# ndefilippis/SWRaytracing

Measured on AMD Instinct MI355X. Metric: packet-steps/sec @ 512² field, 1e6 packets; 1/2/4/8-GPU scaling, higher is better.
Workload: dtype f64

## Files before the change

### swraytracing_amd/csrc/swrt_host_packets.hpp

```cpp
#pragma once
#include <algorithm>
#include <vector>

#include "swrt_ctx.hpp"
#include "swrt_host_fields.hpp"
#include "swrt_bin.hpp"
#include "swrt_kernels.hpp"
#include "swrt_tile.hpp"
#include "swrt_share.hpp"
#include "swrt_xka.hpp"
#include "swrt_spectral.hpp"

namespace {

bool use_tile_kernel(const swrt_ctx* c) {
  if (c->rebin_every <= 0) return false;
  if (c->kernel == 2) return true;
  return c->kernel == 0 && c->slot[0].nx >= 2 * kTile;
}

bool tile_binned(const swrt_ctx* c) { return use_tile_kernel(c) && c->bin.tiled_for(tiles_per_side(c->slot[0].nx)); }

struct IvLaunch {
  int nint;
  FieldView views[kMaxIntervals + 1];
  double dts[kMaxIntervals];
  bool div_free;
};

template <typename F, typename... Args>
void launch_k(swrt_ctx* c, F kernel, dim3 grid, dim3 block, Args... args) {
  hipEvent_t stop = c->kev1 ? c->kev1 : (slot_events(c) ? c->use_ev.get() : nullptr);
  hipExtLaunchKernelGGL(kernel, grid, block, 0, c->stream, c->kev0, stop, 0, args...);
  c->tail_ev = stop;
}

constexpr int64_t kMultiStreamFrom = 65536;

int hz_tile_launch(swrt_ctx* c, const TileArgs& t, const TileShare* parts, int nparts, bool zero_counts,
                   bool fork = true) {
  HazardChecker h = c->hz;
  if (zero_counts) {
    const uint64_t tm = h.op(0);
    if (!h.access(0, tm, t.next_counts, kHzWrite, HzRegion::all(), "the next-binning counts' memset"))
      return fail(c, SWRT_ERR_STATE, h.err);
  }
  if (nparts > 1 && fork) {
    h.record(c->fork_ev.get(), 0);
    for (int i = 1; i < nparts; ++i) h.wait(i, c->fork_ev.get());
  }
  const StepArgs& a = t.s;
  for (int p = 0; p < nparts; ++p) {
    const uint64_t tp = h.op(p);
    const HzRegion r = HzRegion::of_share(h.epoch, parts[p]);
    const char* what = t.src ? "a part of the sort launch after a re-binning" : "a part launch";
    const HzRegion rin = t.src ? HzRegion::all() : r;
    bool ok = h.access(p, tp, a.x, kHzRead, rin, what) && h.access(p, tp, a.k, kHzRead, rin, what) &&
              h.access(p, tp, a.perm, kHzRead, rin, what) && h.access(p, tp, t.src, kHzRead, r, what) &&
              h.access(p, tp, t.starts, kHzRead, HzRegion::all(), what) &&
              h.access(p, tp, t.order, kHzRead, HzRegion::all(), what) &&
              h.access(p, tp, t.x_out, kHzWrite, r, what) && h.access(p, tp, t.k_out, kHzWrite, r, what) &&
              h.access(p, tp, t.perm_out, kHzWrite, r, what) &&
              h.access(p, tp, t.next_keys, kHzWrite, r, what) &&
              h.access(p, tp, t.next_counts, kHzAtomic, HzRegion::all(), what) &&
              h.access(p, tp, a.hist_x, kHzWrite, r, what) && h.access(p, tp, a.hist_k, kHzWrite, r, what);
    if (!ok) return fail(c, SWRT_ERR_STATE, h.err);
  }
  c->hz = std::move(h);
  return SWRT_OK;
}

int launch_tiles(swrt_ctx* c, void (*kernel)(TileArgs), int nt, TileArgs t, bool zero_counts) {
  const int ntiles = t.ntx * t.ntx;
  const int S = c->n >= kMultiStreamFrom ? c->packet_streams : 1;
  const bool skew = c->dbg.share_skew && t.next_keys != nullptr;
  if (skew && !c->hz.on) return fail(c, SWRT_ERR_STATE, "the skewed share runs only under the hazard checker");
  const bool multi = S == 2 && c->stream == c->stream0.get() && c->sx[0].get() != nullptr &&
                     (skew ? ntiles % 8 == 0 && ntiles / 8 >= 3 : ntiles % 16 == 0);
  if (!multi) {
    t.sh = TileShare{ntiles, -1, 1, kShareEven};
    HIPCHK_RC(join_b(c));
    if (c->hz.on) HIPCHK_RC(hz_tile_launch(c, t, &t.sh, 1, zero_counts));
    if (zero_counts) HIPCHK(c, hipMemsetAsync(t.next_counts, 0, sizeof(int) * ntiles, c->stream));
    launch_k(c, kernel, dim3((unsigned)share_grid(t.sh)), dim3(nt), t);
    c->s0_dirty = true;
    return SWRT_OK;
  }
  const TileShare sh[2] = {TileShare{ntiles, 0, 2, skew ? kShareSkew : kShareEven},
                           TileShare{ntiles, 1, 2, skew ? kShareSkew : kShareEven}};
  const bool fork = c->s0_dirty || zero_counts || skew;
  if (c->hz.on) HIPCHK_RC(hz_tile_launch(c, t, sh, 2, zero_counts, fork));
  if (zero_counts) HIPCHK(c, hipMemsetAsync(t.next_counts, 0, sizeof(int) * ntiles, c->stream));
  if (fork) {
    HIPCHK(c, hipEventRecord(c->fork_ev.get(), c->stream));
    HIPCHK(c, hipStreamWaitEvent(c->sx[0].get(), c->fork_ev.get(), 0));
  }
  c->s0_dirty = false;
  t.sh = sh[0];
  hipExtLaunchKernelGGL(kernel, dim3((unsigned)share_grid(sh[0])), dim3(nt), 0, c->stream, c->kev0, nullptr, 0, t);
  if (c->dbg.spin_us > 0)
    hipLaunchKernelGGL(debug_spin_kernel, dim3(1), dim3(64), 0, c->sx[0].get(), (c->dbg.spin_us + 3) / 4);
  t.sh = sh[1];
  hipExtLaunchKernelGGL(kernel, dim3((unsigned)share_grid(sh[1])), dim3(nt), 0, c->sx[0].get(), nullptr, c->kev1, 0, t);
  c->b_pending = 1;
  c->tail_ev = nullptr;
  return SWRT_OK;
}

bool sparse_tiles(const swrt_ctx* c, int64_t ntiles) {
  if (c->sparse_mode == 1) return false;
  if (c->sparse_mode == 2) return true;
  return c->n < (int64_t)kSparseBelow * ntiles;
}

int tile_threads(const swrt_ctx* c, bool v5_two, int64_t ntiles) {
  return v5_two && sparse_tiles(c, ntiles) ? kSparseThreads : kTileThreads;
}

bool two_v5(const swrt_ctx* c, int nslots, int sa) {
  bool v5 = nslots >= 2;
  for (int i = 0; i < nslots && v5; ++i) v5 = c->slot[sa + i].div_free;
  return v5;
}

int tile_cells(const swrt_ctx* c, int64_t nx) {
  if (use_tile_kernel(c)) return kTile;
  if (c->tile > 0) return (int)std::min<int64_t>(c->tile, nx);
  int t = 8;
  while ((nx + t - 1) / t > 64) t *= 2;
  return t;
}

using LeapKernel = void (*)(StepArgs);
LeapKernel leap_kernel(int nslots) { return nslots == 2 ? leapfrog_kernel<true> : leapfrog_kernel<false>; }

int rebin(swrt_ctx* c, bool indirect, int tile = 0, int lanes = kTileThreads) {
  if (int rc = join_b(c)) return rc;
  c->s0_dirty = true;
  const Slot& s = c->slot[0];
  const FieldView v = view_of(s);
  BinGeom g;
  g.dx = v.dx; g.px = v.px; g.py = v.py; g.inv_px = v.inv_px; g.inv_py = v.inv_py; g.inv_dx = v.inv_dx;
  g.nx = v.nx;
  g.tile = tile > 0 ? tile : tile_cells(c, s.nx);
  g.ntx = (int)((s.nx + g.tile - 1) / g.tile);
  const int nbins = g.ntx * g.ntx;
  if (nbins > kMaxBins) return fail(c, SWRT_ERR_ARG, "too many spatial bins (raise tile size)");
  const int64_t n = c->n;
  const unsigned grid = nblocks(n, 256 * kBinPerThread);
  const bool keys_valid = c->bin.keys_valid_for(nbins, v.nx, v.dx);
  const PacketSet &in = c->pk.cur, &out = c->pk.out;
  if (c->hz.on) {
    HazardChecker& h = c->hz;
    const uint64_t t = h.op(0);
    const char* what = "a re-binning";
    const bool ok =
        hz_whole(h, t, kHzRead, what, {in.x.get(), in.k.get(), in.perm.get()}) &&
        hz_whole(h, t, keys_valid ? kHzRead : kHzWrite, what, {c->keys.get()}) &&
        hz_whole(h, t, kHzWrite, what, {c->bins.counts(), c->bins.cursor(), c->bins.starts(), c->bins.tile_order()}) &&
        (indirect ? hz_whole(h, t, kHzWrite, what, {c->src_idx.get()})
                  : hz_whole(h, t, kHzWrite, what, {out.x.get(), out.k.get(), out.perm.get()}));
    if (!ok) return fail(c, SWRT_ERR_STATE, h.err);
    ++h.epoch;
  }
  if (!keys_valid) {
    if (c->bin.needs_count_memset(nbins))
      HIPCHK(c, hipMemsetAsync(c->bins.counts(), 0, sizeof(int) * nbins, c->stream));
    hipLaunchKernelGGL(bin_count_kernel, dim3(grid), dim3(256), sizeof(int) * nbins, c->stream, g, in.x.get(), n,
                       nbins, c->keys.get(), c->bins.counts());
    HIPCHK(c, hipGetLastError());
  }
  if (c->dbg.corrupt_count != 0) {
    hipLaunchKernelGGL(debug_corrupt_count_kernel, dim3(1), dim3(64), 0, c->stream, c->bins.counts(), nbins / 2,
                       c->dbg.corrupt_count);
    c->dbg.corrupt_count = 0;
  }
  hipLaunchKernelGGL(bin_scan_kernel, dim3(1), dim3(1024), 0, c->stream, c->bins.counts(), nbins, c->bins.cursor(),
                     c->bins.starts(), n, c->dev_err.dev(), c->bins.tile_order(), lanes);
  HIPCHK(c, hipGetLastError());
  hipLaunchKernelGGL(indirect ? bin_scatter_kernel<true> : bin_scatter_kernel<false>, dim3(grid), dim3(256),
                     2 * sizeof(int) * nbins, c->stream, in.x.get(), in.k.get(), in.perm.get(), c->keys.get(), n, nbins,
                     c->bins.cursor(), out.x.get(), out.k.get(), out.perm.get(), indirect ? c->src_idx.get() : nullptr);
  HIPCHK(c, hipGetLastError());
  if (!indirect) c->pk.flip();
  c->bin.rebinned(nbins, g.tile, lanes, indirect);
  return SWRT_OK;
}

struct TileKernel { void (*fn)(TileArgs); int threads; };
TileKernel tile_kernel_of(bool two, bool v5, bool fma, bool sparse) {
  constexpr int T = kTile, M = kMargin, NT = kTileThreads, ST = kSparseThreads, PF = kSparsePrefetch;
  constexpr int MW = kSparseMinWaves;
  if (two && v5 && sparse)
    return {fma ? tile_leapfrog_kernel<true, T, M, ST, true, true, PF, MW>
                : tile_leapfrog_kernel<true, T, M, ST, true, false, PF, MW>, ST};
  if (two && v5) return {fma ? tile_leapfrog_kernel<true, T, M, NT, true, true> : tile_leapfrog_kernel<true, T, M, NT, true>, NT};
  if (two) return {tile_leapfrog_kernel<true, T, M, NT>, NT};
  if (v5) return {fma ? tile_leapfrog_kernel<false, T, M, NT, true, true> : tile_leapfrog_kernel<false, T, M, NT, true>, NT};
  return {tile_leapfrog_kernel<false, T, M, NT>, NT};
}

int tile_launch(swrt_ctx* c, const StepArgs& a, bool count_next, const IvLaunch* iv = nullptr) {
  TileArgs t;
  t.s = a;
  t.ivmode = iv != nullptr;
  t.nint = iv ? iv->nint : 1;
  if (iv) {
    for (int i = 0; i <= iv->nint; ++i) t.ivn[i] = iv->views[i].nodes;
    for (int i = 0; i < iv->nint; ++i) t.ivdt[i] = iv->dts[i];
  }
  t.x_out = c->pk.out.x.get();
  t.k_out = c->pk.out.k.get();
  t.perm_out = c->pk.out.perm.get();
  t.starts = c->bins.starts();
  t.order = c->bins.tile_order();
  if (c->bin.tile() != kTile) return fail(c, SWRT_ERR_STATE, "the binning is not the LDS-tiled kernel's");
  t.ntx = tiles_per_side(a.f0.nx);
  const int ntiles = t.ntx * t.ntx;
  t.next_keys = nullptr;
  t.next_counts = nullptr;
  t.sort_cells = c->bin.cells_sorted() ? 0 : 1;
  t.src = nullptr;
  t.sort_lead = c->sort_lead ? 0.5 * a.dt * (double)std::max<int64_t>(1, c->rebin_every) : 0.0;
  if (c->bin.src_pending()) {
    t.src = c->src_idx.get();
    t.sort_cells = 1;
  }
  bool zero = false;
  if (count_next && ntiles == c->bin.nbins()) {
    zero = !c->bin.counts_zero();
    t.next_keys = c->keys.get();
    t.next_counts = c->bins.counts();
  }
  const bool two = a.nslots == 2;
  const bool v5 = two ? (iv ? iv->div_free : two_v5(c, 2, 0)) : c->slot[0].div_free;
  const TileKernel tk = tile_kernel_of(two, v5, c->gather_mode == 1,
                                       two && v5 && tile_threads(c, true, ntiles) == kSparseThreads);
  HIPCHK_RC(launch_tiles(c, tk.fn, tk.threads, t, zero));
  HIPCHK(c, hipGetLastError());
  c->bin.tile_launched(t.next_keys != nullptr, a.f0.nx, a.f0.dx);
  if (t.src != nullptr && c->b_pending && !c->dbg.legacy_park) {
    c->pk.park_cur();
  } else {
    c->pk.flip();
  }
  return SWRT_OK;
}

int leap_launch(swrt_ctx* c, const StepArgs& a, unsigned grid) {
  HIPCHK_RC(join_b(c));
  c->s0_dirty = true;
  if (c->hz.on) {
    HazardChecker& h = c->hz;
    const uint64_t t = h.op(0);
    const char* what = "the per-packet leapfrog launch";
    if (!(hz_whole(h, t, kHzWrite, what, {a.x, a.k}) && hz_whole(h, t, kHzRead, what, {a.perm}) &&
          hz_whole(h, t, kHzWrite, what, {a.hist_x, a.hist_k})))
      return fail(c, SWRT_ERR_STATE, h.err);
  }
  c->bin.per_packet_launched();
  if (c->kev1) {
    launch_k(c, leap_kernel(a.nslots), dim3(grid), dim3(256), a);
  } else {
    hipLaunchKernelGGL(leap_kernel(a.nslots), dim3(grid), dim3(256), 0, c->stream, a);
    c->tail_ev = nullptr;
  }
  HIPCHK(c, hipGetLastError());
  return SWRT_OK;
}

int timed_launch(swrt_ctx* c, const StepArgs& a, unsigned grid, bool count_next, const IvLaunch* iv = nullptr) {
  const bool timed = c->timing_every > 0 && (c->launch_count++ % c->timing_every) == 0;
  const auto launch = [&] { return use_tile_kernel(c) ? tile_launch(c, a, count_next, iv) : leap_launch(c, a, grid); };
  if (!timed) return launch();
  if (c->timing.used + 2 > kMaxEvents) {
    if (int rc = sync_sx(c)) return rc;
    HIPCHK(c, hipStreamSynchronize(c->stream));
    for (size_t i = 0; i + 1 < c->timing.used; i += 2) {
      float ms = 0.f;
      HIPCHK(c, hipEventElapsedTime(&ms, c->timing.ev[i].get(), c->timing.ev[i + 1].get()));
      c->timing.folded_ms += ms;
      c->timing.folded_n += 1;
    }
    c->timing.used = 0;
  }
  if (c->timing.used + 2 > c->timing.ev.size()) {
    for (int e = 0; e < 64; ++e) {
      Event ev;
      HIPCHK(c, ev.create(hipEventDefault));
      c->timing.ev.push_back(std::move(ev));
    }
  }
  c->kev0 = c->timing.ev[c->timing.used].get();
  c->kev1 = c->timing.ev[c->timing.used + 1].get();
  c->timing.used += 2;
  const int rc = launch();
  c->kev0 = c->kev1 = nullptr;
  return rc;
}

int leap_rebin_if_due(swrt_ctx* c, int nslots, int sa) {
  if (c->rebin_every <= 0) return SWRT_OK;
  const bool tiled = use_tile_kernel(c);
  const int64_t ntx = tiles_per_side(c->slot[sa].nx), ntiles = tiled ? ntx * ntx : 0;
  const int lanes = tiled ? tile_threads(c, two_v5(c, nslots, sa), ntiles) : kTileThreads;
  if (c->bin.due(c->rebin_every) || (tiled && (c->bin.tile() != kTile || c->bin.lanes() != lanes)))
    return rebin(c, tiled, tiled ? kTile : 0, lanes);
  return SWRT_OK;
}

StepArgs step_args(swrt_ctx* c, const FieldView& f0, const FieldView& f1, int nslots, double dt, double f, double gH,
                   double alpha0, double dalpha, double bump, int64_t save_every) {
  StepArgs a;
  a.f0 = f0;
  a.f1 = f1;
  a.nslots = nslots;
  a.n = c->n;
  a.dt = dt;
  a.half = dt / 2;
  a.f2 = f * f;
  a.fastdisp = dispersion_fast(a.f2);
  a.gH = gH;
  a.alpha0 = alpha0;
  a.dalpha = dalpha;
  a.bump = bump;
  a.save_every = save_every > 0 ? save_every : 1;
  a.hist_x = save_every > 0 ? c->hist.a.get() : nullptr;
  a.hist_k = save_every > 0 ? c->hist.b.get() : nullptr;
  a.frame0 = c->hist.ext.frames();
  return a;
}

int advance_launch(swrt_ctx* c, StepArgs& a, int64_t s0, int64_t nsteps, int64_t steps, const IvLaunch* iv = nullptr) {
  a.x = c->pk.cur.x.get();
  a.k = c->pk.cur.k.get();
  a.perm = c->pk.cur.perm.get();
  a.s0 = s0;
  a.nsteps = (int)nsteps;
  const bool count_next = c->rebin_every > 0 && steps >= c->bin.steps_left(c->rebin_every);
  slot_writes_wait(c);
  HIPCHK_RC(timed_launch(c, a, nblocks(c->n, 256), count_next, iv));
  c->bin.stepped(steps);
  return SWRT_OK;
}

int run_advance(swrt_ctx* c, double dt, int64_t nsteps, double f, double gH, int nslots,
                double alpha0, double dalpha, double bump, int64_t save_every, int sa = 0) {
  const FieldView f0 = view_of(c->slot[sa]);
  StepArgs a = step_args(c, f0, nslots == 2 ? view_of(c->slot[sa + 1]) : f0, nslots, dt, f, gH, alpha0, dalpha, bump,
                         save_every);
  int64_t s0 = 0;
  while (s0 < nsteps) {
    int64_t chunk = std::min<int64_t>(kMaxStepsPerLaunch, nsteps - s0);
    HIPCHK_RC(leap_rebin_if_due(c, nslots, sa));
    if (c->rebin_every > 0) chunk = std::min<int64_t>(chunk, c->bin.steps_left(c->rebin_every));
    HIPCHK_RC(advance_launch(c, a, s0, chunk, chunk));
    s0 += chunk;
  }
  return SWRT_OK;
}

int run_advance_intervals(swrt_ctx* c, int nint, const double* hs, int64_t nsub, double f, double gH,
                          double alpha0, double dalpha, double bump, int64_t save_every) {
  const bool fused = use_tile_kernel(c) && c->rebin_every > 0 && c->rebin_every % nsub == 0 &&
                     nsub <= kMaxStepsPerLaunch;
  const int64_t fpi = save_every > 0 ? nsub / save_every : 0;
  int i0 = 0;
  while (i0 < nint) {
    int k = 0;
    if (fused) {
      HIPCHK_RC(leap_rebin_if_due(c, std::min(nint - i0, kMaxIntervals) + 1, i0));
      k = (int)std::min<int64_t>({(int64_t)(nint - i0), c->bin.steps_left(c->rebin_every) / nsub,
                                  (int64_t)kMaxIntervals});
    }
    if (k < 1) {
      HIPCHK_RC(run_advance(c, hs[i0], nsub, f, gH, 2, alpha0, dalpha, bump, save_every, i0));
      c->hist.ext.committed(fpi);
      i0 += 1;
      continue;
    }
    IvLaunch iv;
    iv.nint = k;
    iv.div_free = true;
    for (int i = 0; i <= k; ++i) {
      iv.views[i] = view_of(c->slot[i0 + i]);
      iv.div_free = iv.div_free && c->slot[i0 + i].div_free;
    }
    for (int i = 0; i < k; ++i) iv.dts[i] = hs[i0 + i];
    StepArgs a = step_args(c, iv.views[0], iv.views[1], 2, hs[i0], f, gH, alpha0, dalpha, bump, save_every);
    HIPCHK_RC(advance_launch(c, a, 0, nsub, k * nsub, &iv));
    c->hist.ext.committed(k * fpi);
    i0 += k;
  }
  return SWRT_OK;
}

int ensure_history(swrt_ctx* c, int64_t new_frames) {
  const int64_t per = 2 * c->n;
  if (c->hist.ext.fits(new_frames, per)) return SWRT_OK;
  if (int rc = join_b(c)) return rc;
  c->s0_dirty = true;
  const double *old_x = c->hist.a.get(), *old_k = c->hist.b.get();
  HIPCHK_RC(series_reserve(c, c->hist, per, per, new_frames, 0, "history allocation failed"));
  if (c->hz.on) {
    c->hz.bufs.erase(old_x);
    c->hz.bufs.erase(old_k);
    c->hz.name(c->hist.a.get(), "history x frames");
    c->hz.name(c->hist.b.get(), "history k frames");
  }
  return SWRT_OK;
}

auto xka_tile_kernel_of(int tile) {
  return tile == 8 ? xka_tile_kernel<8, kXkaMargin, 256> : xka_tile_kernel<16, kXkaMargin, 256>;
}
auto spectral_eval_kernel_of(int precision) {
  return precision == 64 ? spectral_eval_kernel<double> : spectral_eval_kernel<float>;
}
auto spectral_leapfrog_kernel_of(int precision) {
  return precision == 64 ? spectral_leapfrog_kernel<double> : spectral_leapfrog_kernel<float>;
}
}
```

### swraytracing_amd/csrc/swrt_tile.hpp

```cpp
#pragma once
#include <hip/hip_runtime.h>
#include <stdint.h>

#include "swrt_kernels.hpp"

namespace swrt {

struct TileArgs {
  StepArgs s;
  double* x_out;
  double* k_out;
  int* perm_out;
  const int* starts;
  const int* order;
  int ntx;
  int* next_keys;
  int* next_counts;
  int sort_cells;
  const int* src;
  double sort_lead;
  TileShare sh;
  int ivmode;
  int nint;
  const double* ivn[kMaxIntervals + 1];
  double ivdt[kMaxIntervals];
};

__device__ __forceinline__ const double* iv_nodes(const TileArgs& ta, int i) {
  const double* p = ta.ivn[0];
#pragma unroll
  for (int j = 1; j <= kMaxIntervals; ++j)
    if (i == j) p = ta.ivn[j];
  return p;
}
__device__ __forceinline__ double iv_dt(const TileArgs& ta, int i) {
  double d = ta.ivdt[0];
#pragma unroll
  for (int j = 1; j < kMaxIntervals; ++j)
    if (i == j) d = ta.ivdt[j];
  return d;
}

__device__ __forceinline__ int wg_work_range(const int* starts, const int* order, int64_t n, const TileShare& sh,
                                             int& pbeg, int& pend) {
  int tile = share_slot(sh, (int)blockIdx.x);
  if (order != nullptr) tile = order[tile];
  const int nn = (int)n;
  pbeg = min(max(starts[tile], 0), nn);
  pend = min(max(starts[tile + 1], pbeg), nn);
  return tile;
}
__device__ __forceinline__ int wg_work_range(const int* starts, int64_t n, int& pbeg, int& pend) {
  TileShare sh;
  sh.ntiles = (int)gridDim.x;
  return wg_work_range(starts, nullptr, n, sh, pbeg, pend);
}

__device__ __forceinline__ int wg_work(const TileArgs& ta, int& pbeg, int& pend) {
  return wg_work_range(ta.starts, ta.order, ta.s.n, ta.sh, pbeg, pend);
}

__device__ __forceinline__ int ring_diff(int a, int b, int n) {
  int d = a - b;
  if (d >= n / 2) d -= n;
  if (d < -n / 2) d += n;
  return d;
}

__device__ __forceinline__ int b128_lane_rank(int lane) {
  const int h = lane & 32, t = lane & 31;
  int k;
  if (t < 4) k = t;
  else if (t < 12) k = 16 + (t - 4);
  else if (t < 16) k = 4 + (t - 12);
  else if (t < 20) k = 24 + (t - 16);
  else if (t < 28) k = 8 + (t - 20);
  else k = t;
  return h + k;
}

template <bool TWO>
struct Tap6 {
  double2 a0, a1, a2, b0, b1, b2;
};
template <bool TWO, int WN>
__device__ __forceinline__ void tap6_read(const double2* p, int e, Tap6<TWO>& t) {
  t.a0 = p[0 * WN + e];
  t.a1 = p[1 * WN + e];
  t.a2 = p[2 * WN + e];
  if constexpr (TWO) {
    t.b0 = p[3 * WN + e];
    t.b1 = p[4 * WN + e];
    t.b2 = p[5 * WN + e];
  }
}
template <bool TWO, int W, int WN>
__device__ __forceinline__ void gather6_lds(const double2* lds, int node0, const Stencil& s,
                                            double o0[kRec], double o1[kRec]) {
#pragma unroll
  for (int f = 0; f < kRec; ++f) { o0[f] = -0.0; o1[f] = -0.0; }
  const double2* p = lds + node0;
  double wx[kNT], wy[kNT];
#pragma unroll
  for (int q = 0; q < kNT; ++q) {
    wx[q] = s.wx[q];
    wy[q] = s.wy[q];
    asm volatile("" : "+v"(wx[q]));
    asm volatile("" : "+v"(wy[q]));
  }
  if constexpr (TWO) {
#pragma unroll
    for (int i = 0; i < kNT; ++i) {
#pragma unroll
      for (int j = 0; j < kNT; ++j) {
        const int e = i * W + j;
        const double wij = wx[i] * wy[j];
        const double2 a0 = p[0 * WN + e], a1 = p[1 * WN + e], a2 = p[2 * WN + e];
        o0[0] = o0[0] + wij * a0.x; o0[1] = o0[1] + wij * a0.y;
        o0[2] = o0[2] + wij * a1.x; o0[3] = o0[3] + wij * a1.y;
        o0[4] = o0[4] + wij * a2.x; o0[5] = o0[5] + wij * a2.y;
        const double2 b0 = p[3 * WN + e], b1 = p[4 * WN + e], b2 = p[5 * WN + e];
        o1[0] = o1[0] + wij * b0.x; o1[1] = o1[1] + wij * b0.y;
        o1[2] = o1[2] + wij * b1.x; o1[3] = o1[3] + wij * b1.y;
        o1[4] = o1[4] + wij * b2.x; o1[5] = o1[5] + wij * b2.y;
      }
    }
    return;
  }
  Tap6<TWO> cur, nxt;
  tap6_read<TWO, WN>(p, 0, cur);
#pragma unroll
  for (int t = 0; t < kNT * kNT; ++t) {
    const int i = t / kNT, j = t % kNT;
    if (t + 1 < kNT * kNT) tap6_read<TWO, WN>(p, ((t + 1) / kNT) * W + (t + 1) % kNT, nxt);
    if constexpr (!TWO) __builtin_amdgcn_sched_barrier(0);
    const double wij = wx[i] * wy[j];
    o0[0] = o0[0] + wij * cur.a0.x; o0[1] = o0[1] + wij * cur.a0.y;
    o0[2] = o0[2] + wij * cur.a1.x; o0[3] = o0[3] + wij * cur.a1.y;
    o0[4] = o0[4] + wij * cur.a2.x; o0[5] = o0[5] + wij * cur.a2.y;
    if constexpr (TWO) {
      o1[0] = o1[0] + wij * cur.b0.x; o1[1] = o1[1] + wij * cur.b0.y;
      o1[2] = o1[2] + wij * cur.b1.x; o1[3] = o1[3] + wij * cur.b1.y;
      o1[4] = o1[4] + wij * cur.b2.x; o1[5] = o1[5] + wij * cur.b2.y;
    }
    if constexpr (!TWO) __builtin_amdgcn_sched_barrier(0);
    if (t + 1 < kNT * kNT) cur = nxt;
  }
}

template <bool TWO>
struct Tap5 {
  double2 a0, a1, c, b0, b1;
};
template <bool TWO, int WN>
__device__ __forceinline__ void tap5_read(const double2* p, int e, Tap5<TWO>& t) {
  t.a0 = p[0 * WN + e];
  t.a1 = p[1 * WN + e];
  if constexpr (TWO) {
    t.c = p[2 * WN + e];
    t.b0 = p[3 * WN + e];
    t.b1 = p[4 * WN + e];
  } else {
    t.c.x = reinterpret_cast<const double*>(p + 2 * WN + e)[0];
  }
}
template <bool TWO, int W, int WN, bool FMA = false, int PF = 1>
__device__ __forceinline__ void gather5_lds(const double2* lds, int node0, const Stencil& s,
                                            double o0[kRec], double o1[kRec]) {
  static_assert(PF >= 1 && PF <= 4, "prefetch depth");
  constexpr int NTAP = kNT * kNT;
#pragma unroll
  for (int f = 0; f < 5; ++f) { o0[f] = -0.0; o1[f] = -0.0; }
  const double2* p = lds + node0;
  double wx[kNT], wy[kNT];
#pragma unroll
  for (int q = 0; q < kNT; ++q) {
    wx[q] = s.wx[q];
    wy[q] = s.wy[q];
    asm volatile("" : "+v"(wx[q]));
    asm volatile("" : "+v"(wy[q]));
  }
  Tap5<TWO> ring[PF + 1];
#pragma unroll
  for (int t = 0; t < PF; ++t) tap5_read<TWO, WN>(p, (t / kNT) * W + t % kNT, ring[t]);
#pragma unroll
  for (int t = 0; t < NTAP; ++t) {
    const int i = t / kNT, j = t % kNT;
    if (t + PF < NTAP) tap5_read<TWO, WN>(p, ((t + PF) / kNT) * W + (t + PF) % kNT, ring[(t + PF) % (PF + 1)]);
    __builtin_amdgcn_sched_barrier(0);
    const Tap5<TWO>& cur = ring[t % (PF + 1)];
    const double wij = wx[i] * wy[j];
    o0[0] = madd<FMA>(o0[0], wij, cur.a0.x); o0[1] = madd<FMA>(o0[1], wij, cur.a0.y);
    o0[2] = madd<FMA>(o0[2], wij, cur.a1.x); o0[3] = madd<FMA>(o0[3], wij, cur.a1.y);
    o0[4] = madd<FMA>(o0[4], wij, cur.c.x);
    if constexpr (TWO) {
      o1[0] = madd<FMA>(o1[0], wij, cur.b0.x); o1[1] = madd<FMA>(o1[1], wij, cur.b0.y);
      o1[2] = madd<FMA>(o1[2], wij, cur.b1.x); o1[3] = madd<FMA>(o1[3], wij, cur.b1.y);
      o1[4] = madd<FMA>(o1[4], wij, cur.c.y);
    }
    __builtin_amdgcn_sched_barrier(0);
  }
  o0[5] = -o0[2];
  o1[5] = -o1[2];
}

template <bool TWO, int T, int M, int NT, int WS = T + 5 + 2 * M, bool V5 = false>
__device__ __forceinline__ void stage_window_regs(const FieldView& f0, const FieldView& f1, int ox, int oy,
                                                  double2* win) {
  constexpr int W = T + 5 + 2 * M;
  constexpr int WN = W * WS;
  const int nx = f0.nx, npad = f0.npad;
  for (int e = threadIdx.x; e < W * W; e += NT) {
    const int wi = e / W, wj = e % W;
    int gx = (ox - M - 2 + wi) % nx; gx += gx < 0 ? nx : 0;
    int gy = (oy - M - 2 + wj) % nx; gy += gy < 0 ? nx : 0;
    const size_t src = ((size_t)(gx + kPadLo) * npad + (gy + kPadLo)) * kRec;
    const int d = wi * WS + wj;
    const double2* s0 = reinterpret_cast<const double2*>(f0.nodes + src);
    if constexpr (V5 && TWO) {
      const double2* s1 = reinterpret_cast<const double2*>(f1.nodes + src);
      const double2 a0 = s0[0], a1 = s0[1], a2 = s0[2], b0 = s1[0], b1 = s1[1], b2 = s1[2];
      win[0 * WN + d] = a0;
      win[1 * WN + d] = a1;
      win[2 * WN + d] = make_double2(a2.x, b2.x);
      win[3 * WN + d] = b0;
      win[4 * WN + d] = b1;
    } else {
      win[0 * WN + d] = s0[0];
      win[1 * WN + d] = s0[1];
      win[2 * WN + d] = s0[2];
      if constexpr (TWO) {
        const double2* s1 = reinterpret_cast<const double2*>(f1.nodes + src);
        win[3 * WN + d] = s1[0];
        win[4 * WN + d] = s1[1];
        win[5 * WN + d] = s1[2];
      }
    }
  }
}

#ifdef SWRT_PHASE_TIMING
__device__ unsigned long long swrt_phase_dbg[16384 * 8];
#define SWRT_STAMP(slot)                                                            \
  do {                                                                              \
    if (tid == 0) swrt_phase_dbg[blockIdx.x * 8 + (slot)] = __builtin_amdgcn_s_memrealtime(); \
  } while (0)
#else
#define SWRT_STAMP(slot) \
  do {                   \
  } while (0)
#endif

#ifndef SWRT_TILE_MIN_WAVES
#define SWRT_TILE_MIN_WAVES 4
#endif

template <bool TWO, int T, int M, int NT, bool V5 = false, bool FMA = false, int PF = 1,
          int MINW = SWRT_TILE_MIN_WAVES>
__global__ void __launch_bounds__(NT, MINW) tile_leapfrog_kernel(TileArgs ta) {
  static_assert(!FMA || V5, "the FMA gather exists for the five-sum window only");
  constexpr int W = T + 5 + 2 * M;
  constexpr int WS = W + ((12 - W % 16) + 16) % 16;
  constexpr int WNP = W * WS;
  constexpr int NCH = TWO ? (V5 ? 5 : 6) : 3;
  constexpr int NB = T * T + 1;
  constexpr int MAXB = 2 * NT;
  __shared__ double2 win[NCH * WNP];
  __shared__ int hist[NB];
  __shared__ int kr[MAXB];
  __shared__ int order[MAXB];
  __shared__ int nbr[9];
#ifdef SWRT_PHASE_TIMING
  __shared__ int nfall;
  __shared__ unsigned simds;
#endif

  const StepArgs& a = ta.s;
  const int tid = threadIdx.x;
  int pbeg, pend;
  const int tile = wg_work(ta, pbeg, pend);
  const int tx = tile / ta.ntx, ty = tile % ta.ntx;
  const int nx = a.f0.nx, npad = a.f0.npad;
  const int ox = tx * T, oy = ty * T;
  const int oxm = ((ox - M) % nx + nx) % nx, oym = ((oy - M) % nx + nx) % nx;
  if (tid < 9) nbr[tid] = 0;
#ifdef SWRT_PHASE_TIMING
  if (tid == 0) nfall = 0;
  if (tid == 0) simds = 0;
#endif
  SWRT_STAMP(0);
#ifdef SWRT_PHASE_TIMING
  if (tid == 0) {
    unsigned hw, xcc;
    asm volatile("s_getreg_b32 %0, hwreg(HW_REG_HW_ID)" : "=s"(hw));
    asm volatile("s_getreg_b32 %0, hwreg(HW_REG_XCC_ID)" : "=s"(xcc));
    swrt_phase_dbg[blockIdx.x * 8 + 7] = ((unsigned long long)xcc << 32) | hw;
    swrt_phase_dbg[blockIdx.x * 8 + 6] = (unsigned long long)(pend - pbeg);
  }
  __syncthreads();
  if ((tid & 63) == 0) {
    unsigned hw;
    asm volatile("s_getreg_b32 %0, hwreg(HW_REG_HW_ID)" : "=s"(hw));
    atomicOr(&simds, ((hw >> 4) & 3u) << (2 * (tid >> 6)));
  }
  __syncthreads();
  if (tid == 0) swrt_phase_dbg[blockIdx.x * 8 + 6] |= (unsigned long long)simds << 32;
#endif

  const int lane_rank = b128_lane_rank(tid & 63);
  const int nint = ta.ivmode ? ta.nint : 1;
  for (int ivl = 0; ivl < nint; ++ivl) {
  FieldView fa = a.f0, fb = a.f1;
  if (ta.ivmode) {
    fa.nodes = iv_nodes(ta, ivl);
    fb.nodes = iv_nodes(ta, ivl + 1);
  }
  const double dt = ta.ivmode ? iv_dt(ta, ivl) : a.dt;
  const double half = ta.ivmode ? 0.5 * dt : a.half;
  const bool first = ivl == 0;
  const double* xin = first ? a.x : ta.x_out;
  const double* kin = first ? a.k : ta.k_out;
  const int* pin = first ? a.perm : ta.perm_out;
  const int sortc = first ? ta.sort_cells : 0;
  const int* srcp = first ? ta.src : nullptr;
  int* nkeys = ivl == nint - 1 ? ta.next_keys : nullptr;
  const int64_t sbase = a.s0 + (int64_t)ivl * a.nsteps;
  if (!first) __syncthreads();

  stage_window_regs<TWO, T, M, NT, WS, V5>(fa, fb, ox, oy, win);
  if (!sortc) {
    __syncthreads();
    SWRT_STAMP(1);
  }
  for (int b0 = pbeg; b0 < pend; b0 += MAXB) {
    const int nb = min(MAXB, pend - b0);
    if (sortc) {
    for (int h = tid; h < NB; h += NT) hist[h] = 0;
    __syncthreads();
    if (b0 == pbeg) SWRT_STAMP(1);
    for (int i = tid; i < nb; i += NT) {
      const int64_t p = srcp ? srcp[b0 + i] : b0 + i;
      double xs = xin[p], ys = xin[a.n + p];
      if (ta.sort_lead != 0.0) {
        const double kx = kin[p], ky = kin[a.n + p];
        const double s = ta.sort_lead * a.gH / sqrt(a.f2 + a.gH * (kx * kx + ky * ky));
        xs += s * kx;
        ys += s * ky;
      }
      const int ic = fast_cell(xs, a.f0.inv_dx, nx);
      const int jc = fast_cell(ys, a.f0.inv_dx, nx);
      const int dx_ = min(max(ring_diff(ic, ox, nx), 0), T - 1);
      const int dy_ = min(max(ring_diff(jc, oy, nx), 0), T - 1);
      int key;
      if constexpr (T == 16) {
        key = (dx_ >= 0 && dx_ < T && dy_ >= 0 && dy_ < T)
                  ? ((dy_ & 1) | ((dx_ & 1) << 1) | ((dy_ & 2) << 1) | ((dx_ & 2) << 2) |
                     ((dy_ & 4) << 2) | ((dx_ & 4) << 3) | ((dy_ & 8) << 3) | ((dx_ & 8) << 4))
                  : T * T;
      } else {
        key = 0;
#pragma unroll
        for (int b = 0; (1 << b) < T; ++b) key |= (((dy_ >> b) & 1) << (2 * b)) | (((dx_ >> b) & 1) << (2 * b + 1));
      }
      const int r = atomicAdd(&hist[key], 1);
      kr[i] = (key << 16) | r;
    }
    __syncthreads();
    if (tid < 64) {
      constexpr int PER = (NB + 63) / 64;
      int loc[PER];
      int sum = 0;
#pragma unroll
      for (int q = 0; q < PER; ++q) {
        const int h = tid * PER + q;
        loc[q] = h < NB ? hist[h] : 0;
        sum += loc[q];
      }
      int incl = sum;
#pragma unroll
      for (int off = 1; off < 64; off <<= 1) {
        const int v = __shfl_up(incl, off, 64);
        if (tid >= off) incl += v;
      }
      int run = incl - sum;
#pragma unroll
      for (int q = 0; q < PER; ++q) {
        const int h = tid * PER + q;
        if (h < NB) hist[h] = run;
        run += loc[q];
      }
    }
    __syncthreads();
    for (int i = tid; i < nb; i += NT) {
      const int v = kr[i];
      order[hist[v >> 16] + (v & 0xffff)] = srcp ? srcp[b0 + i] : b0 + i;
    }
    __syncthreads();
    }
    if (b0 == pbeg) SWRT_STAMP(2);

    for (int r0 = tid & ~63; r0 < nb; r0 += NT) {
      const int r = r0 + lane_rank;
      if (r >= nb) continue;
      const int64_t pi = sortc ? order[r] : b0 + r;
      const int64_t po = b0 + r;
      double x0 = xin[pi], y0 = xin[a.n + pi];
      double k0 = kin[pi], l0 = kin[a.n + pi];
      const int orig = pin[pi];
      double hcx, hcy;
      drift_inc(k0, l0, a.f2, a.gH, half, a.fastdisp, hcx, hcy);
      double sgd = (double)(ta.ivmode ? (int64_t)0 : sbase);
      for (int st = 0; st < a.nsteps; ++st) {
        const int64_t sg = sbase + st;
        const double alpha = a.alpha0 + sgd * a.dalpha;
        sgd = sgd + 1.0;
        const double x1 = x0 + hcx;
        const double y1 = y0 + hcy;
        Stencil sc;
        stencil_at(a.f0, x1, y1, a.bump, sc);
        const int d0 = sc.ic - oxm, d1 = sc.jc - oym;
        const unsigned ux = min((unsigned)d0, (unsigned)(d0 + nx)), uy = min((unsigned)d1, (unsigned)(d1 + nx));
        double I[kRec], J[kRec];
        const bool inwin = max(ux, uy) < (unsigned)(T + 2 * M);
#ifdef SWRT_PHASE_TIMING
        if (!inwin) atomicAdd(&nfall, 1);
#endif
        if (inwin) {
          if constexpr (V5)
            gather5_lds<TWO, WS, WNP, FMA, PF>(win, (int)(ux * WS + uy), sc, I, J);
          else
            gather6_lds<TWO, WS, WNP>(win, (int)(ux * WS + uy), sc, I, J);
        } else {
          gather6_lean<TWO, FMA>(fa.nodes, fb.nodes, npad, sc, I, J);
        }
        if constexpr (TWO) {
          const double oma = 1 - alpha;
#pragma unroll
          for (int q = 0; q < (V5 ? 5 : kRec); ++q) I[q] = madd<FMA>(oma * I[q], alpha, J[q]);
          if constexpr (V5) I[5] = -I[2];
        }
        const double x2 = x1 + dt * I[0];
        const double y2 = y1 + dt * I[1];
        const double k2 = k0 - dt * (I[2] * k0 + I[4] * l0);
        const double l2 = l0 - dt * (I[3] * k0 + I[5] * l0);
        drift_inc(k2, l2, a.f2, a.gH, half, a.fastdisp, hcx, hcy);
        x0 = x2 + hcx;
        y0 = y2 + hcy;
        k0 = k2;
        l0 = l2;
        if (a.hist_x != nullptr && ((sg + 1) % a.save_every) == 0) {
          const int64_t fr = a.frame0 + (sg + 1) / a.save_every - 1;
          double* hx = a.hist_x + fr * 2 * a.n;
          double* hk = a.hist_k + fr * 2 * a.n;
          hx[orig] = x0; hx[a.n + orig] = y0;
          hk[orig] = k0; hk[a.n + orig] = l0;
        }
      }
      ta.x_out[po] = x0; ta.x_out[a.n + po] = y0;
      ta.k_out[po] = k0; ta.k_out[a.n + po] = l0;
      ta.perm_out[po] = orig;
      if (nkeys != nullptr) {
        const int ic = fast_cell(x0, a.f0.inv_dx, nx);
        const int jc = fast_cell(y0, a.f0.inv_dx, nx);
        const int ntx_ = ta.ntx;
        const int ntx2 = ic / T, nty2 = jc / T;
        nkeys[po] = ntx2 * ntx_ + nty2;
        const int ddx = ring_diff(ntx2, tx, ntx_), ddy = ring_diff(nty2, ty, ntx_);
        if (ddx != 0 || ddy != 0) {
          atomicAdd(&nbr[4], -1);
          if (ddx >= -1 && ddx <= 1 && ddy >= -1 && ddy <= 1)
            atomicAdd(&nbr[(ddx + 1) * 3 + (ddy + 1)], 1);
          else
            atomicAdd(&ta.next_counts[ntx2 * ntx_ + nty2], 1);
        }
      }
    }
    __syncthreads();
    if (b0 == pbeg) SWRT_STAMP(3);
  }
  }
  if (ta.next_keys != nullptr) {
    __syncthreads();
    const int v = tid < 9 ? nbr[tid] + (tid == 4 ? pend - pbeg : 0) : 0;
    if (v != 0) {
      const int n_ = ta.ntx;
      const int gx = ((tx + tid / 3 - 1) % n_ + n_) % n_, gy = ((ty + tid % 3 - 1) % n_ + n_) % n_;
      atomicAdd(&ta.next_counts[gx * n_ + gy], v);
    }
  }
  SWRT_STAMP(4);
#ifdef SWRT_PHASE_TIMING
  __syncthreads();
  if (tid == 0) swrt_phase_dbg[blockIdx.x * 8 + 5] = (unsigned long long)nfall;
#endif
}

}
```

Baseline: 26.39 billion.

## Specialize tile kernel on history/multi-interval and cut register pressure

Adds HIST and MULTI template flags so the common launch compiles without history saving or interval looping. Kernel arguments are reloaded from the kernarg segment instead of being held live in registers. Tile and range values are made wave-uniform with readfirstlane. The per-batch cell sort moves into a helper, and the window staging is reorganised into row-per-thread-column passes with 32-bit offsets. The aim is lower VGPR/SGPR pressure, cheaper address math and fewer barriers, at the cost of more template instantiations and more complex index logic.

```diff
diff --git a/swraytracing_amd/csrc/swrt_host_packets.hpp b/swraytracing_amd/csrc/swrt_host_packets.hpp
--- a/swraytracing_amd/csrc/swrt_host_packets.hpp
+++ b/swraytracing_amd/csrc/swrt_host_packets.hpp
@@ -188,16 +188,24 @@
 }
 
 struct TileKernel { void (*fn)(TileArgs); int threads; };
+template <bool X>
 TileKernel tile_kernel_of(bool two, bool v5, bool fma, bool sparse) {
   constexpr int T = kTile, M = kMargin, NT = kTileThreads, ST = kSparseThreads, PF = kSparsePrefetch;
-  constexpr int MW = kSparseMinWaves;
+  constexpr int MW = kSparseMinWaves, W4 = SWRT_TILE_MIN_WAVES;
   if (two && v5 && sparse)
-    return {fma ? tile_leapfrog_kernel<true, T, M, ST, true, true, PF, MW>
-                : tile_leapfrog_kernel<true, T, M, ST, true, false, PF, MW>, ST};
-  if (two && v5) return {fma ? tile_leapfrog_kernel<true, T, M, NT, true, true> : tile_leapfrog_kernel<true, T, M, NT, true>, NT};
-  if (two) return {tile_leapfrog_kernel<true, T, M, NT>, NT};
-  if (v5) return {fma ? tile_leapfrog_kernel<false, T, M, NT, true, true> : tile_leapfrog_kernel<false, T, M, NT, true>, NT};
-  return {tile_leapfrog_kernel<false, T, M, NT>, NT};
+    return {fma ? tile_leapfrog_kernel<true, T, M, ST, true, true, PF, MW, X, X>
+                : tile_leapfrog_kernel<true, T, M, ST, true, false, PF, MW, X, X>, ST};
+  if (two && v5)
+    return {fma ? tile_leapfrog_kernel<true, T, M, NT, true, true, 1, W4, X, X>
+                : tile_leapfrog_kernel<true, T, M, NT, true, false, 1, W4, X, X>, NT};
+  if (two) return {tile_leapfrog_kernel<true, T, M, NT, false, false, 1, W4, X, X>, NT};
+  if (v5)
+    return {fma ? tile_leapfrog_kernel<false, T, M, NT, true, true, 1, W4, X, X>
+                : tile_leapfrog_kernel<false, T, M, NT, true, false, 1, W4, X, X>, NT};
+  return {tile_leapfrog_kernel<false, T, M, NT, false, false, 1, W4, X, X>, NT};
+}
+TileKernel tile_kernel_of(bool two, bool v5, bool fma, bool sparse, bool hist, bool multi) {
+  return hist || multi ? tile_kernel_of<true>(two, v5, fma, sparse) : tile_kernel_of<false>(two, v5, fma, sparse);
 }
 
 int tile_launch(swrt_ctx* c, const StepArgs& a, bool count_next, const IvLaunch* iv = nullptr) {
@@ -235,7 +243,8 @@
   const bool two = a.nslots == 2;
   const bool v5 = two ? (iv ? iv->div_free : two_v5(c, 2, 0)) : c->slot[0].div_free;
   const TileKernel tk = tile_kernel_of(two, v5, c->gather_mode == 1,
-                                       two && v5 && tile_threads(c, true, ntiles) == kSparseThreads);
+                                       two && v5 && tile_threads(c, true, ntiles) == kSparseThreads,
+                                       a.hist_x != nullptr, iv != nullptr);
   HIPCHK_RC(launch_tiles(c, tk.fn, tk.threads, t, zero));
   HIPCHK(c, hipGetLastError());
   c->bin.tile_launched(t.next_keys != nullptr, a.f0.nx, a.f0.dx);
diff --git a/swraytracing_amd/csrc/swrt_tile.hpp b/swraytracing_amd/csrc/swrt_tile.hpp
--- a/swraytracing_amd/csrc/swrt_tile.hpp
+++ b/swraytracing_amd/csrc/swrt_tile.hpp
@@ -26,6 +26,12 @@
   double ivdt[kMaxIntervals];
 };
 
+__device__ __forceinline__ auto tile_args_again() {
+  auto* p = (const __attribute__((address_space(4))) TileArgs*)__builtin_amdgcn_kernarg_segment_ptr();
+  asm volatile("" : "+s"(p));
+  return p;
+}
+
 __device__ __forceinline__ const double* iv_nodes(const TileArgs& ta, int i) {
   const double* p = ta.ivn[0];
 #pragma unroll
@@ -204,37 +210,66 @@
   o1[5] = -o1[2];
 }
 
+template <bool TWO, int WN, bool V5>
+__device__ __forceinline__ void stage_record(const double2* s0, const double2* s1, int d, double2* win) {
+  if constexpr (V5 && TWO) {
+    const double2 a0 = s0[0], a1 = s0[1], a2 = s0[2], b0 = s1[0], b1 = s1[1], b2 = s1[2];
+    win[0 * WN + d] = a0;
+    win[1 * WN + d] = a1;
+    win[2 * WN + d] = make_double2(a2.x, b2.x);
+    win[3 * WN + d] = b0;
+    win[4 * WN + d] = b1;
+  } else if constexpr (TWO) {
+    const double2 a0 = s0[0], a1 = s0[1], a2 = s0[2], b0 = s1[0], b1 = s1[1], b2 = s1[2];
+    win[0 * WN + d] = a0;
+    win[1 * WN + d] = a1;
+    win[2 * WN + d] = a2;
+    win[3 * WN + d] = b0;
+    win[4 * WN + d] = b1;
+    win[5 * WN + d] = b2;
+  } else {
+    const double2 a0 = s0[0], a1 = s0[1], a2 = s0[2];
+    win[0 * WN + d] = a0;
+    win[1 * WN + d] = a1;
+    win[2 * WN + d] = a2;
+  }
+}
 template <bool TWO, int T, int M, int NT, int WS = T + 5 + 2 * M, bool V5 = false>
 __device__ __forceinline__ void stage_window_regs(const FieldView& f0, const FieldView& f1, int ox, int oy,
                                                   double2* win) {
   constexpr int W = T + 5 + 2 * M;
   constexpr int WN = W * WS;
+  constexpr int CW = W <= 32 ? 32 : (W <= 64 ? 64 : 128);
+  constexpr int RP = NT / CW;
+  static_assert(W <= CW && NT % CW == 0, "window rows per workgroup pass");
   const int nx = f0.nx, npad = f0.npad;
-  for (int e = threadIdx.x; e < W * W; e += NT) {
-    const int wi = e / W, wj = e % W;
-    int gx = (ox - M - 2 + wi) % nx; gx += gx < 0 ? nx : 0;
+  const int wj = (int)threadIdx.x % CW;
+  int wi = (int)threadIdx.x / CW;
+  if (wj >= W) return;
+  const char* n0 = reinterpret_cast<const char*>(f0.nodes);
+  const char* n1 = reinterpret_cast<const char*>(f1.nodes);
+  constexpr unsigned kRecBytes = kRec * sizeof(double);
+  if (nx >= W && (uint64_t)npad * (uint64_t)npad * kRecBytes < (1ull << 32)) {
+    int gy = oy - M - 2 + wj;
+    gy += gy < 0 ? nx : 0;
+    gy -= gy >= nx ? nx : 0;
+    const unsigned col = (unsigned)(gy + kPadLo) * kRecBytes;
+    const unsigned rowb = (unsigned)npad * kRecBytes;
+    for (int d = wi * WS + wj; wi < W; wi += RP, d += RP * WS) {
+      int gx = ox - M - 2 + wi;
+      gx += gx < 0 ? nx : 0;
+      gx -= gx >= nx ? nx : 0;
+      const unsigned off = (unsigned)(gx + kPadLo) * rowb + col;
+      stage_record<TWO, WN, V5>(reinterpret_cast<const double2*>(n0 + off),
+                                reinterpret_cast<const double2*>(n1 + off), d, win);
+    }
+  } else {
     int gy = (oy - M - 2 + wj) % nx; gy += gy < 0 ? nx : 0;
-    const size_t src = ((size_t)(gx + kPadLo) * npad + (gy + kPadLo)) * kRec;
-    const int d = wi * WS + wj;
-    const double2* s0 = reinterpret_cast<const double2*>(f0.nodes + src);
-    if constexpr (V5 && TWO) {
-      const double2* s1 = reinterpret_cast<const double2*>(f1.nodes + src);
-      const double2 a0 = s0[0], a1 = s0[1], a2 = s0[2], b0 = s1[0], b1 = s1[1], b2 = s1[2];
-      win[0 * WN + d] = a0;
-      win[1 * WN + d] = a1;
-      win[2 * WN + d] = make_double2(a2.x, b2.x);
-      win[3 * WN + d] = b0;
-      win[4 * WN + d] = b1;
-    } else {
-      win[0 * WN + d] = s0[0];
-      win[1 * WN + d] = s0[1];
-      win[2 * WN + d] = s0[2];
-      if constexpr (TWO) {
-        const double2* s1 = reinterpret_cast<const double2*>(f1.nodes + src);
-        win[3 * WN + d] = s1[0];
-        win[4 * WN + d] = s1[1];
-        win[5 * WN + d] = s1[2];
-      }
+    for (; wi < W; wi += RP) {
+      int gx = (ox - M - 2 + wi) % nx; gx += gx < 0 ? nx : 0;
+      const size_t off = ((size_t)(gx + kPadLo) * npad + (gy + kPadLo)) * kRecBytes;
+      stage_record<TWO, WN, V5>(reinterpret_cast<const double2*>(n0 + off),
+                                reinterpret_cast<const double2*>(n1 + off), wi * WS + wj, win);
     }
   }
 }
@@ -251,12 +286,89 @@
   } while (0)
 #endif
 
+template <int T, int NT, int NB>
+__device__ __forceinline__ void sort_batch_by_cell(int b0, int nb, bool first_batch, int tile, int* hist,
+                                                   int* kr, int* order) {
+  const auto* g = tile_args_again();
+  int tid = threadIdx.x;
+  asm volatile("" : "+v"(tid));
+  const int nx = g->s.f0.nx;
+  const int tx = (int)((unsigned)tile / (unsigned)g->ntx), ty = tile - tx * g->ntx;
+  const int ox = tx * T, oy = ty * T;
+  const int64_t n = g->s.n;
+  const double* xin = g->s.x;
+  const double* kin = g->s.k;
+  const int* srcp = g->src;
+  const double sort_lead = g->sort_lead, gH = g->s.gH, f2 = g->s.f2, inv_dx = g->s.f0.inv_dx;
+  for (int h = tid; h < NB; h += NT) hist[h] = 0;
+  __syncthreads();
+  if (first_batch) SWRT_STAMP(1);
+  for (int i = tid; i < nb; i += NT) {
+    const int64_t p = srcp ? srcp[b0 + i] : b0 + i;
+    double xs = xin[p], ys = xin[n + p];
+    if (sort_lead != 0.0) {
+      const double kx = kin[p], ky = kin[n + p];
+      const double s = sort_lead * gH / sqrt(f2 + gH * (kx * kx + ky * ky));
+      xs += s * kx;
+      ys += s * ky;
+    }
+    const int ic = fast_cell(xs, inv_dx, nx);
+    const int jc = fast_cell(ys, inv_dx, nx);
+    const int dx_ = min(max(ring_diff(ic, ox, nx), 0), T - 1);
+    const int dy_ = min(max(ring_diff(jc, oy, nx), 0), T - 1);
+    int key;
+    if constexpr (T == 16) {
+      key = (dx_ >= 0 && dx_ < T && dy_ >= 0 && dy_ < T)
+                ? ((dy_ & 1) | ((dx_ & 1) << 1) | ((dy_ & 2) << 1) | ((dx_ & 2) << 2) |
+                   ((dy_ & 4) << 2) | ((dx_ & 4) << 3) | ((dy_ & 8) << 3) | ((dx_ & 8) << 4))
+                : T * T;
+    } else {
+      key = 0;
+#pragma unroll
+      for (int b = 0; (1 << b) < T; ++b) key |= (((dy_ >> b) & 1) << (2 * b)) | (((dx_ >> b) & 1) << (2 * b + 1));
+    }
+    const int r = atomicAdd(&hist[key], 1);
+    kr[i] = (key << 16) | r;
+  }
+  __syncthreads();
+  if (tid < 64) {
+    constexpr int PER = (NB + 63) / 64;
+    int loc[PER];
+    int sum = 0;
+#pragma unroll
+    for (int q = 0; q < PER; ++q) {
+      const int h = tid * PER + q;
+      loc[q] = h < NB ? hist[h] : 0;
+      sum += loc[q];
+    }
+    int incl = sum;
+#pragma unroll
+    for (int off = 1; off < 64; off <<= 1) {
+      const int v = __shfl_up(incl, off, 64);
+      if (tid >= off) incl += v;
+    }
+    int run = incl - sum;
+#pragma unroll
+    for (int q = 0; q < PER; ++q) {
+      const int h = tid * PER + q;
+      if (h < NB) hist[h] = run;
+      run += loc[q];
+    }
+  }
+  __syncthreads();
+  for (int i = tid; i < nb; i += NT) {
+    const int v = kr[i];
+    order[hist[v >> 16] + (v & 0xffff)] = srcp ? srcp[b0 + i] : b0 + i;
+  }
+  __syncthreads();
+}
+
 #ifndef SWRT_TILE_MIN_WAVES
 #define SWRT_TILE_MIN_WAVES 4
 #endif
 
 template <bool TWO, int T, int M, int NT, bool V5 = false, bool FMA = false, int PF = 1,
-          int MINW = SWRT_TILE_MIN_WAVES>
+          int MINW = SWRT_TILE_MIN_WAVES, bool HIST = true, bool MULTI = true>
 __global__ void __launch_bounds__(NT, MINW) tile_leapfrog_kernel(TileArgs ta) {
   static_assert(!FMA || V5, "the FMA gather exists for the five-sum window only");
   constexpr int W = T + 5 + 2 * M;
@@ -278,12 +390,25 @@
   const StepArgs& a = ta.s;
   const int tid = threadIdx.x;
   int pbeg, pend;
-  const int tile = wg_work(ta, pbeg, pend);
-  const int tx = tile / ta.ntx, ty = tile % ta.ntx;
+  const int tile = min(max(__builtin_amdgcn_readfirstlane(wg_work(ta, pbeg, pend)), 0), ta.ntx * ta.ntx - 1);
+  pbeg = __builtin_amdgcn_readfirstlane(pbeg);
+  pend = __builtin_amdgcn_readfirstlane(pend);
   const int nx = a.f0.nx, npad = a.f0.npad;
-  const int ox = tx * T, oy = ty * T;
-  const int oxm = ((ox - M) % nx + nx) % nx, oym = ((oy - M) % nx + nx) % nx;
-  if (tid < 9) nbr[tid] = 0;
+  int ox, oy;
+  {
+    const int tx = (int)((unsigned)tile / (unsigned)ta.ntx), ty = tile - tx * ta.ntx;
+    ox = tx * T;
+    oy = ty * T;
+  }
+  int oxm = ox - M, oym = oy - M;
+  if (nx >= M) {
+    oxm += oxm < 0 ? nx : 0;
+    oym += oym < 0 ? nx : 0;
+  } else {
+    oxm = (oxm % nx + nx) % nx;
+    oym = (oym % nx + nx) % nx;
+  }
+  if (tid < 9) nbr[tid] = tid == 4 ? pend - pbeg : 0;
 #ifdef SWRT_PHASE_TIMING
   if (tid == 0) nfall = 0;
   if (tid == 0) simds = 0;
@@ -307,23 +432,21 @@
   if (tid == 0) swrt_phase_dbg[blockIdx.x * 8 + 6] |= (unsigned long long)simds << 32;
 #endif
 
-  const int lane_rank = b128_lane_rank(tid & 63);
-  const int nint = ta.ivmode ? ta.nint : 1;
+  const unsigned lane_rank = (unsigned)b128_lane_rank(tid & 63);
+  const int wave0 = __builtin_amdgcn_readfirstlane(tid & ~63);
+  const bool ivmode = MULTI && ta.ivmode;
+  const int nint = ivmode ? ta.nint : 1;
   for (int ivl = 0; ivl < nint; ++ivl) {
   FieldView fa = a.f0, fb = a.f1;
-  if (ta.ivmode) {
+  if (ivmode) {
     fa.nodes = iv_nodes(ta, ivl);
     fb.nodes = iv_nodes(ta, ivl + 1);
   }
-  const double dt = ta.ivmode ? iv_dt(ta, ivl) : a.dt;
-  const double half = ta.ivmode ? 0.5 * dt : a.half;
-  const bool first = ivl == 0;
-  const double* xin = first ? a.x : ta.x_out;
-  const double* kin = first ? a.k : ta.k_out;
-  const int* pin = first ? a.perm : ta.perm_out;
+  const double dt = ivmode ? iv_dt(ta, ivl) : a.dt;
+  const double half = ivmode ? 0.5 * dt : a.half;
+  const bool first = !MULTI || ivl == 0;
   const int sortc = first ? ta.sort_cells : 0;
-  const int* srcp = first ? ta.src : nullptr;
-  int* nkeys = ivl == nint - 1 ? ta.next_keys : nullptr;
+  const bool last = !MULTI || ivl == nint - 1;
   const int64_t sbase = a.s0 + (int64_t)ivl * a.nsteps;
   if (!first) __syncthreads();
 
@@ -332,86 +455,41 @@
     __syncthreads();
     SWRT_STAMP(1);
   }
-  for (int b0 = pbeg; b0 < pend; b0 += MAXB) {
-    const int nb = min(MAXB, pend - b0);
-    if (sortc) {
-    for (int h = tid; h < NB; h += NT) hist[h] = 0;
-    __syncthreads();
-    if (b0 == pbeg) SWRT_STAMP(1);
-    for (int i = tid; i < nb; i += NT) {
-      const int64_t p = srcp ? srcp[b0 + i] : b0 + i;
-      double xs = xin[p], ys = xin[a.n + p];
-      if (ta.sort_lead != 0.0) {
-        const double kx = kin[p], ky = kin[a.n + p];
-        const double s = ta.sort_lead * a.gH / sqrt(a.f2 + a.gH * (kx * kx + ky * ky));
-        xs += s * kx;
-        ys += s * ky;
+  const int bstep = sortc ? MAXB : max(pend - pbeg, 1);
+  for (int b0 = pbeg; b0 < pend; b0 += bstep) {
+    const int nb = min(bstep, pend - b0);
+    if (sortc) sort_batch_by_cell<T, NT, NB>(b0, nb, b0 == pbeg, tile, hist, kr, order);
+    if (b0 == pbeg) SWRT_STAMP(2);
+
+    for (int r0 = wave0; r0 < nb; r0 += NT) {
+      const int r = r0 + (int)lane_rank;
+      if (r >= nb) continue;
+      const int64_t slot0 = (int64_t)b0 + r0;
+      double x0, y0, k0, l0;
+      int orig;
+      {
+        const auto* g = tile_args_again();
+        const int64_t n = g->s.n;
+        const double* xi = first ? g->s.x : g->x_out;
+        const double* ki = first ? g->s.k : g->k_out;
+        const int* pi_ = first ? g->s.perm : g->perm_out;
+        if (sortc) {
+          const int64_t pi = order[r];
+          x0 = xi[pi]; y0 = xi[n + pi];
+          k0 = ki[pi]; l0 = ki[n + pi];
+          orig = pi_[pi];
+        } else {
+          const double* xr = xi + slot0;
+          const double* kr_ = ki + slot0;
+          x0 = xr[lane_rank]; y0 = (xr + n)[lane_rank];
+          k0 = kr_[lane_rank]; l0 = (kr_ + n)[lane_rank];
+          orig = (pi_ + slot0)[lane_rank];
+        }
       }
-      const int ic = fast_cell(xs, a.f0.inv_dx, nx);
-      const int jc = fast_cell(ys, a.f0.inv_dx, nx);
-      const int dx_ = min(max(ring_diff(ic, ox, nx), 0), T - 1);
-      const int dy_ = min(max(ring_diff(jc, oy, nx), 0), T - 1);
-      int key;
-      if constexpr (T == 16) {
-        key = (dx_ >= 0 && dx_ < T && dy_ >= 0 && dy_ < T)
-                  ? ((dy_ & 1) | ((dx_ & 1) << 1) | ((dy_ & 2) << 1) | ((dx_ & 2) << 2) |
-                     ((dy_ & 4) << 2) | ((dx_ & 4) << 3) | ((dy_ & 8) << 3) | ((dx_ & 8) << 4))
-                  : T * T;
-      } else {
-        key = 0;
-#pragma unroll
-        for (int b = 0; (1 << b) < T; ++b) key |= (((dy_ >> b) & 1) << (2 * b)) | (((dx_ >> b) & 1) << (2 * b + 1));
-      }
-      const int r = atomicAdd(&hist[key], 1);
-      kr[i] = (key << 16) | r;
-    }
-    __syncthreads();
-    if (tid < 64) {
-      constexpr int PER = (NB + 63) / 64;
-      int loc[PER];
-      int sum = 0;
-#pragma unroll
-      for (int q = 0; q < PER; ++q) {
-        const int h = tid * PER + q;
-        loc[q] = h < NB ? hist[h] : 0;
-        sum += loc[q];
-      }
-      int incl = sum;
-#pragma unroll
-      for (int off = 1; off < 64; off <<= 1) {
-        const int v = __shfl_up(incl, off, 64);
-        if (tid >= off) incl += v;
-      }
-      int run = incl - sum;
-#pragma unroll
-      for (int q = 0; q < PER; ++q) {
-        const int h = tid * PER + q;
-        if (h < NB) hist[h] = run;
-        run += loc[q];
-      }
-    }
-    __syncthreads();
-    for (int i = tid; i < nb; i += NT) {
-      const int v = kr[i];
-      order[hist[v >> 16] + (v & 0xffff)] = srcp ? srcp[b0 + i] : b0 + i;
-    }
-    __syncthreads();
-    }
-    if (b0 == pbeg) SWRT_STAMP(2);
-
-    for (int r0 = tid & ~63; r0 < nb; r0 += NT) {
-      const int r = r0 + lane_rank;
-      if (r >= nb) continue;
-      const int64_t pi = sortc ? order[r] : b0 + r;
-      const int64_t po = b0 + r;
-      double x0 = xin[pi], y0 = xin[a.n + pi];
-      double k0 = kin[pi], l0 = kin[a.n + pi];
-      const int orig = pin[pi];
       double hcx, hcy;
       drift_inc(k0, l0, a.f2, a.gH, half, a.fastdisp, hcx, hcy);
-      double sgd = (double)(ta.ivmode ? (int64_t)0 : sbase);
+      double sgd = (double)(ivmode ? (int64_t)0 : sbase);
       for (int st = 0; st < a.nsteps; ++st) {
-        const int64_t sg = sbase + st;
         const double alpha = a.alpha0 + sgd * a.dalpha;
         sgd = sgd + 1.0;
         const double x1 = x0 + hcx;
@@ -431,7 +509,12 @@
           else
             gather6_lds<TWO, WS, WNP>(win, (int)(ux * WS + uy), sc, I, J);
         } else {
-          gather6_lean<TWO, FMA>(fa.nodes, fb.nodes, npad, sc, I, J);
+          if constexpr (MULTI) {
+            gather6_lean<TWO, FMA>(fa.nodes, fb.nodes, npad, sc, I, J);
+          } else {
+            const auto* g = tile_args_again();
+            gather6_lean<TWO, FMA>(g->s.f0.nodes, g->s.f1.nodes, g->s.f0.npad, sc, I, J);
+          }
         }
         if constexpr (TWO) {
           const double oma = 1 - alpha;
@@ -448,21 +531,32 @@
         y0 = y2 + hcy;
         k0 = k2;
         l0 = l2;
-        if (a.hist_x != nullptr && ((sg + 1) % a.save_every) == 0) {
-          const int64_t fr = a.frame0 + (sg + 1) / a.save_every - 1;
-          double* hx = a.hist_x + fr * 2 * a.n;
-          double* hk = a.hist_k + fr * 2 * a.n;
-          hx[orig] = x0; hx[a.n + orig] = y0;
-          hk[orig] = k0; hk[a.n + orig] = l0;
+        if constexpr (HIST) {
+          const int64_t sg = sbase + st;
+          if (a.hist_x != nullptr && ((sg + 1) % a.save_every) == 0) {
+            const int64_t fr = a.frame0 + (sg + 1) / a.save_every - 1;
+            double* hx = a.hist_x + fr * 2 * a.n;
+            double* hk = a.hist_k + fr * 2 * a.n;
+            hx[orig] = x0; hx[a.n + orig] = y0;
+            hk[orig] = k0; hk[a.n + orig] = l0;
+          }
         }
       }
-      ta.x_out[po] = x0; ta.x_out[a.n + po] = y0;
-      ta.k_out[po] = k0; ta.k_out[a.n + po] = l0;
-      ta.perm_out[po] = orig;
-      if (nkeys != nullptr) {
-        const int ic = fast_cell(x0, a.f0.inv_dx, nx);
-        const int jc = fast_cell(y0, a.f0.inv_dx, nx);
-        const int ntx_ = ta.ntx;
+      const auto* g = tile_args_again();
+      const int64_t n = g->s.n;
+      double* xw = g->x_out + slot0;
+      double* kw = g->k_out + slot0;
+      xw[lane_rank] = x0; (xw + n)[lane_rank] = y0;
+      kw[lane_rank] = k0; (kw + n)[lane_rank] = l0;
+      (g->perm_out + slot0)[lane_rank] = orig;
+      int* nkeys = g->next_keys;
+      if (last && nkeys != nullptr) {
+        const int64_t po = slot0 + lane_rank;
+        const int nxk = g->s.f0.nx;
+        const int ic = fast_cell(x0, a.f0.inv_dx, nxk);
+        const int jc = fast_cell(y0, a.f0.inv_dx, nxk);
+        const int ntx_ = g->ntx;
+        const int tx = (int)((unsigned)tile / (unsigned)ntx_), ty = tile - tx * ntx_;
         const int ntx2 = ic / T, nty2 = jc / T;
         nkeys[po] = ntx2 * ntx_ + nty2;
         const int ddx = ring_diff(ntx2, tx, ntx_), ddy = ring_diff(nty2, ty, ntx_);
@@ -471,21 +565,29 @@
           if (ddx >= -1 && ddx <= 1 && ddy >= -1 && ddy <= 1)
             atomicAdd(&nbr[(ddx + 1) * 3 + (ddy + 1)], 1);
           else
-            atomicAdd(&ta.next_counts[ntx2 * ntx_ + nty2], 1);
+            atomicAdd(&g->next_counts[ntx2 * ntx_ + nty2], 1);
         }
       }
     }
+#ifdef SWRT_PHASE_TIMING
     __syncthreads();
+#else
+    if (sortc) __syncthreads();
+#endif
     if (b0 == pbeg) SWRT_STAMP(3);
   }
   }
-  if (ta.next_keys != nullptr) {
+  const auto* g = tile_args_again();
+  if (g->next_keys != nullptr) {
     __syncthreads();
-    const int v = tid < 9 ? nbr[tid] + (tid == 4 ? pend - pbeg : 0) : 0;
+    int t9 = tid;
+    asm volatile("" : "+v"(t9));
+    const int v = t9 < 9 ? nbr[t9] : 0;
     if (v != 0) {
-      const int n_ = ta.ntx;
-      const int gx = ((tx + tid / 3 - 1) % n_ + n_) % n_, gy = ((ty + tid % 3 - 1) % n_ + n_) % n_;
-      atomicAdd(&ta.next_counts[gx * n_ + gy], v);
+      const int n_ = g->ntx;
+      const int tx = (int)((unsigned)tile / (unsigned)n_), ty = tile - tx * n_;
+      const int gx = ((tx + t9 / 3 - 1) % n_ + n_) % n_, gy = ((ty + t9 % 3 - 1) % n_ + n_) % n_;
+      atomicAdd(&g->next_counts[gx * n_ + gy], v);
     }
   }
   SWRT_STAMP(4);
```

New measurement: 26.68 billion, median of 6. 1.01x the previous value.
